# pennneutrinos/chroma

Hardware: AMD Instinct MI355X
Metric: photons/sec (propagate_hit) (higher is better)
Workload: dtype f32

## Files before the change

### chroma_amd/csrc/chroma_hip.hip

```cpp
#include <hip/hip_runtime.h>
#include <stdint.h>
#include <stdio.h>
#include <stdarg.h>
#include <stdlib.h>
#include <string.h>
#include <string>
#include <vector>
#include <algorithm>
#include <chrono>
#include <atomic>
#include <mutex>
#include <unordered_map>
#include <map>

#include <dlfcn.h>
#include <rccl/rccl.h>

#ifndef CHROMA_EXPERIMENTAL
#define CHROMA_EXPERIMENTAL 0
#endif
#include "propagate_device.h"
#include "wide_build.h"
#include "host_utils.h"

// ... 466 lines not shown
{
    const uint32_t i = blockIdx.x * blockDim.x + threadIdx.x;
    if (i >= nnodes) return;
    uint4 n = nodes[i];
    if ((n.w >> CHROMA_CHILD_BITS) == 0) { const uint32_t t = n.w & ~CHROMA_NCHILD_MASK; n.w = t < ntriangles ? tri_to_dev[t] : n.w; }
    out[i] = n;
}
__global__ void k_triangle_records(const float *vertices, const uint32_t *triangles, const uint32_t *codes, const uint32_t *rank,
                                   const uint32_t *dev_to_tri, uint32_t nrecords, float4 *tri)
{
    const uint32_t k = blockIdx.x * blockDim.x + threadIdx.x;
    if (k >= nrecords) return;
    const uint32_t t = dev_to_tri[k];
    const uint32_t extra[3] = {codes[t], t, rank[t]};
#pragma unroll
    for (int c = 0; c < 3; c++) {
        const float *vv = vertices + 3 * (size_t)triangles[3 * (size_t)t + c];
        tri[(size_t)TRI_STRIDE * k + c] = make_float4(vv[0], vv[1], vv[2], __uint_as_float(extra[c]));
    }
}
__global__ void k_triangle_phys(GeoView g, uint32_t nrecords, uint4 *out)
{
    const uint32_t k = blockIdx.x * blockDim.x + threadIdx.x;
    if (k >= nrecords) return;
    const float4 *t = g.tri + (size_t)TRI_STRIDE * k;
    const float4 a = t[0], b = t[1], c = t[2];
    const v3 v0 = mk3(a.x, a.y, a.z), v1 = mk3(b.x, b.y, b.z), v2 = mk3(c.x, c.y, c.z);
    const v3 n = triangle_normal(v0, v1, v2);
    uint32_t bx, by, bz;
    leaf_words(g, v0, v1, v2, bx, by, bz);
    out[2 * (size_t)k] = make_uint4(__float_as_uint(n.x), __float_as_uint(n.y), __float_as_uint(n.z), __float_as_uint(a.w));
    out[2 * (size_t)k + 1] = make_uint4(__float_as_uint(b.w), bx, by, bz);
}
__global__ void k_stack_need_ref(const uint4 *nodes, uint32_t nnodes, uint32_t *need, uint32_t *changed)
{
    const uint32_t i = blockIdx.x * blockDim.x + threadIdx.x;
    if (i >= nnodes) return;
    const uint32_t w = nodes[i].w, nchild = w >> CHROMA_CHILD_BITS, first = w & ~CHROMA_NCHILD_MASK;
    if (nchild == 0) return;
    uint32_t best = 0;
    if ((uint64_t)first + nchild > nnodes || first <= i) best = 0xFFFFu;
    else {
        uint32_t rank = 0;
        for (uint32_t j = 0; j < nchild; j++)
            if ((nodes[first + j].w >> CHROMA_CHILD_BITS) != 0) { best = max(best, rank + need[first + j]); rank++; }
        best = min(max(best, rank), 0xFFFFu);
    }
    if (best != need[i]) { need[i] = best; *changed = 1u; }
}
__global__ void k_stack_need_wide(const uint4 *wnodes, uint32_t nwide, uint32_t *need, uint32_t *changed)
{
    const uint32_t i = blockIdx.x * blockDim.x + threadIdx.x;
    if (i >= nwide) return;
    uint32_t inner = 0, below = 0;
    for (int j = 0; j < 8; j++) {
        const uint32_t w = wnodes[8 * (size_t)i + j].w;
        if (w == 0xFFFFFFFFu || (w & 0x80000000u)) continue;
        inner++;
        if (w < nwide && w > i) below = max(below, need[w]);
    }
    const uint32_t v = min(0xFFFFu, inner ? inner - 1u + below : 0u);
    if (v != need[i]) { need[i] = v; *changed = 1u; }
}
template <class Pass>
static int stack_need_fixed_point(chroma_ctx *ctx, size_t n, Pass pass, uint32_t *result)
{
// ... 629 lines not shown
        void *dtri = nullptr;
        size_t bytes = nrecords * (16 * TRI_STRIDE);
        hipError_t e = ctx_malloc(ctx, &dtri, bytes);
        if (e != hipSuccess) { chroma_geometry_destroy(g); return set_error((int)e, "hipMalloc(%zu) for triangle records: %s", bytes, hipGetErrorString(e)); }
        g->allocations.push_back(dtri);
        g->device_bytes += bytes;
        uint32_t *d_rank = nullptr;
        e = ctx_malloc(ctx, (void **)&d_rank, std::max<size_t>(d->ntriangles, 1) * 4);
        if (e != hipSuccess) { chroma_geometry_destroy(g); return set_error((int)e, "hipMalloc for triangle ranks: %s", hipGetErrorString(e)); }
        rc = chroma_internal_htod(ctx, d_rank, tri_rank, (size_t)d->ntriangles * 4);
        if (rc == CHROMA_OK) {
            hipLaunchKernelGGL(k_triangle_records, dim3((unsigned)((nrecords + 255) / 256)), dim3(256), 0, ctx->stream, (const float *)g->d_vertices, (const uint32_t *)g->d_triangles,
                               (const uint32_t *)g->d_material_codes, d_rank, v.dev_to_tri, (uint32_t)nrecords, (float4 *)dtri);
            e = hipStreamSynchronize(ctx->stream);
            if (e != hipSuccess) rc = set_error((int)e, "triangle records: %s", hipGetErrorString(e));
        }
        hipFree(d_rank);
        if (rc != CHROMA_OK) { chroma_geometry_destroy(g); return rc; }
        v.tri = (const float4 *)dtri;
    }
    {
        void *dphys = nullptr;
        size_t bytes = std::max<size_t>(nrecords, 1) * 32;
        hipError_t e = ctx_malloc(ctx, &dphys, bytes);
        if (e != hipSuccess) { chroma_geometry_destroy(g); return set_error((int)e, "hipMalloc(%zu) for physics records: %s", bytes, hipGetErrorString(e)); }
        g->allocations.push_back(dphys);
        g->device_bytes += bytes;
        if (nrecords) hipLaunchKernelGGL(k_triangle_phys, dim3((unsigned)((nrecords + 255) / 256)), dim3(256), 0, ctx->stream, v, (uint32_t)nrecords, (uint4 *)dphys);
        e = hipStreamSynchronize(ctx->stream);
        if (e == hipSuccess) e = hipGetLastError();
        if (e != hipSuccess) { chroma_geometry_destroy(g); return set_error((int)e, "physics records: %s", hipGetErrorString(e)); }
        v.tri_phys = (const uint4 *)dphys;
    }
    phase("triangle records");
    { const uint32_t *p; if ((rc = upload(g, d->colors, d->colors ? d->ntriangles : 0, &p)) != CHROMA_OK) { chroma_geometry_destroy(g); return rc; } g->d_colors = (void *)p; }
    UP(solid_id_map, d->solid_id_map, d->solid_id_map ? d->ntriangles : 0);
    size_t wn = d->wavelength_n;
    UP(mat_refractive_index, d->mat_refractive_index, d->nmaterials * wn);
    UP(mat_absorption_length, d->mat_absorption_length, d->nmaterials * wn);
    UP(mat_scattering_length, d->mat_scattering_length, d->nmaterials * wn);
    UP(mat_num_comp, d->mat_num_comp, d->nmaterials);
    UP(mat_comp_offset, d->mat_comp_offset, d->nmaterials);
    UP(comp_reemission_prob, d->comp_reemission_prob, d->ncomp_total * wn);
    UP(comp_reemission_wvl_cdf, d->comp_reemission_wvl_cdf, d->ncomp_total * wn);
    UP(comp_absorption_length, d->comp_absorption_length, d->ncomp_total * wn);
    UP(comp_reemission_time_cdf, d->comp_reemission_time_cdf, (size_t)d->ncomp_total * d->time_n);
    UP(surf_detect, d->surf_detect, d->nsurfaces * wn);
    UP(surf_absorb, d->surf_absorb, d->nsurfaces * wn);
    UP(surf_reemit, d->surf_reemit, d->nsurfaces * wn);
    UP(surf_reflect_diffuse, d->surf_reflect_diffuse, d->nsurfaces * wn);
    UP(surf_reflect_specular, d->surf_reflect_specular, d->nsurfaces * wn);
    UP(surf_eta, d->surf_eta, d->nsurfaces * wn);
    UP(surf_k, d->surf_k, d->nsurfaces * wn);
    UP(surf_reemission_cdf, d->surf_reemission_cdf, d->nsurfaces * wn);
    {
        std::vector<SurfaceInfo> info(std::max<uint32_t>(d->nsurfaces, 1));
        for (uint32_t s = 0; s < d->nsurfaces; s++)
            info[s] = SurfaceInfo{d->surf_model[s], d->surf_transmissive[s], d->surf_thickness[s],
                                  d->surf_dichroic_index ? d->surf_dichroic_index[s] : -1};
        UP(surf_info, info.data(), info.size());
    }
    UP(dichroic_nangles, d->dichroic_nangles, d->ndichroic);
    UP(dichroic_offset, d->dichroic_offset, d->ndichroic);
    UP(dichroic_angles, d->dichroic_angles, d->ndichroic_angles_total);
    UP(dichroic_reflect, d->dichroic_reflect, d->ndichroic_angles_total * wn);
    UP(dichroic_transmit, d->dichroic_transmit, d->ndichroic_angles_total * wn);
// ... 33 lines not shown
    if (g->stack_need > STACK_LDS + STACK_SCRATCH) {
        uint32_t need = g->stack_need;
        chroma_geometry_destroy(g);
        return set_error(CHROMA_ERR_STACK, "BVH needs %u traversal stack entries, more than the %d supported", need, STACK_LDS + STACK_SCRATCH);
    }
    *out = g;
    return CHROMA_OK;
}

int chroma_geometry_destroy(chroma_geometry *g)
{
    if (!g) return CHROMA_OK;
    hipSetDevice(g->ctx->device);
    hipStreamSynchronize(g->ctx->stream);
    for (void *p : g->allocations) hipFree(p);
    delete g;
    return CHROMA_OK;
}

int chroma_geometry_device_ptr(chroma_geometry *g, const char *name, void **d_ptr, size_t *nbytes)
{
    if (!g || !name || !d_ptr) return set_error(CHROMA_ERR_INVALID, "bad argument");
    std::string n(name);
    size_t bytes = 0; void *p = nullptr;
    if (n == "nodes") { p = g->d_nodes_api; bytes = g->nnodes * 16; }
    else if (n == "vertices") { p = g->d_vertices; bytes = g->nvertices * 12; }
    else if (n == "triangles") { p = g->d_triangles; bytes = g->ntriangles * 12; }
    else if (n == "material_codes") { p = g->d_material_codes; bytes = g->ntriangles * 4; }
    else if (n == "colors") { p = g->d_colors; bytes = g->ntriangles * 4; }
    else if (n == "solid_id_map") { p = (void *)g->view.solid_id_map; bytes = g->ntriangles * 4; }
    else if (n == "solid_id_to_channel_index") { p = (void *)g->view.solid_id_to_channel_index; bytes = (size_t)g->view.nsolids * 4; }
    else if (n == "triangle_records") { p = (void *)g->view.tri; bytes = g->nrecords * (16 * TRI_STRIDE); }
    else if (n == "triangle_phys") { p = (void *)g->view.tri_phys; bytes = g->nrecords * 32; }
    else if (n == "wide_nodes") { p = (void *)g->view.wnodes; bytes = g->nwide * 128; }
    else if (n == "tri_to_dev") { p = (void *)g->view.tri_to_dev; bytes = g->ntriangles * 4; }
    else if (n == "dev_to_tri") { p = (void *)g->view.dev_to_tri; bytes = g->nrecords * 4; }
    else return set_error(CHROMA_ERR_INVALID, "unknown geometry array '%s'", name);
    *d_ptr = p;
    if (nbytes) *nbytes = bytes;
    return CHROMA_OK;
}

int chroma_geometry_stack_need(chroma_geometry *g, uint32_t *entries)
{
    if (!g || !entries) return set_error(CHROMA_ERR_INVALID, "bad argument");
    *entries = g->stack_need;
    return CHROMA_OK;
}

int chroma_propagate_step(chroma_ctx *ctx, chroma_geometry *geom, int32_t first_photon, int32_t nthreads,
                          const uint32_t *d_input_queue, uint32_t *d_output_queue, chroma_rng rng,
                          const chroma_photon_arrays *photons, int32_t max_steps, int32_t use_weights,
                          int32_t scatter_first)
{
    if (!ctx || !geom) return set_error(CHROMA_ERR_INVALID, "bad argument");
    int rc = check_photons(photons, true);
    if (rc) return rc;
    if (first_photon < 0 || nthreads < 0) return set_error(CHROMA_ERR_INVALID, "negative photon range");
    return launch_propagate(ctx, call_opts(ctx), geom, to_view(photons), first_photon, nthreads, d_input_queue, d_output_queue, rng,
                            max_steps, use_weights, scatter_first);
}

int chroma_photon_duplicate(chroma_ctx *ctx, int32_t first_photon, int32_t nthreads,
                            const chroma_photon_arrays *photons, int32_t copies, int32_t stride)
{
    if (!ctx) return set_error(CHROMA_ERR_INVALID, "null ctx");
// ... 908 lines not shown
```

### chroma_amd/csrc/device_common.h

```cpp
#pragma once

#include <hip/hip_runtime.h>
#include <stdint.h>

#define CM_FN __host__ __device__ static inline
#include "../../include/chroma_math.h"
#include "../../include/chroma_hip.h"

#define WAVE 64

struct v3 { float x, y, z; };
__device__ inline v3 mk3(float x, float y, float z) { return v3{x, y, z}; }
__device__ inline v3 operator-(v3 a) { return mk3(-a.x, -a.y, -a.z); }
__device__ inline v3 operator+(v3 a, v3 b) { return mk3(a.x + b.x, a.y + b.y, a.z + b.z); }
__device__ inline v3 operator-(v3 a, v3 b) { return mk3(a.x - b.x, a.y - b.y, a.z - b.z); }
__device__ inline v3 operator*(v3 a, float c) { return mk3(a.x * c, a.y * c, a.z * c); }
__device__ inline v3 operator*(float c, v3 a) { return mk3(c * a.x, c * a.y, c * a.z); }
__device__ inline v3 operator/(v3 a, float c) { return mk3(a.x / c, a.y / c, a.z / c); }
__device__ inline v3 operator/(v3 a, v3 b) { return mk3(a.x / b.x, a.y / b.y, a.z / b.z); }
__device__ inline v3 operator/(float c, v3 a) { return mk3(c / a.x, c / a.y, c / a.z); }
__device__ inline float dot(v3 a, v3 b) { return a.x * b.x + a.y * b.y + a.z * b.z; }
__device__ inline v3 cross(v3 a, v3 b)
{ return mk3(a.y * b.z - a.z * b.y, a.z * b.x - a.x * b.z, a.x * b.y - a.y * b.x); }
__device__ inline float norm(v3 a) { return cm_sqrtf(dot(a, a)); }
__device__ inline v3 normalize(v3 a) { return a / norm(a); }

__device__ inline v3 load3(const float *p, size_t i) { return mk3(p[3 * i], p[3 * i + 1], p[3 * i + 2]); }
__device__ inline void store3(float *p, size_t i, v3 v) { p[3 * i] = v.x; p[3 * i + 1] = v.y; p[3 * i + 2] = v.z; }

struct SurfaceInfo { uint32_t model; uint32_t transmissive; float thickness; int32_t dichroic_index; };

#ifndef TRI_STRIDE
#define TRI_STRIDE 3
#endif
struct GeoView {
    const uint4  *nodes;
    const uint4  *wnodes;
    const float4 *tri;
    const uint4  *tri_phys;
    const uint32_t *tri_to_dev, *dev_to_tri;
    const float *mat_refractive_index, *mat_absorption_length, *mat_scattering_length;
    const uint32_t *mat_num_comp, *mat_comp_offset;
    const float *comp_reemission_prob, *comp_reemission_wvl_cdf, *comp_absorption_length, *comp_reemission_time_cdf;
    const float *surf_detect, *surf_absorb, *surf_reemit, *surf_reflect_diffuse, *surf_reflect_specular,
                *surf_eta, *surf_k, *surf_reemission_cdf;
    const SurfaceInfo *surf_info;
    const uint32_t *dichroic_nangles, *dichroic_offset;
    const float *dichroic_angles, *dichroic_reflect, *dichroic_transmit;
    const uint32_t *solid_id_map;
    const int32_t  *solid_id_to_channel_index;
    float world_origin[3];
    float world_scale;
    float suspect_margin;
    float slab_grow;
    uint32_t wavelength_n; float wavelength_start, wavelength_step;
    uint32_t time_n;       float time_start, time_step;
    uint32_t nnodes, ntriangles, nsolids, nchannels, nwide;
    uint32_t plain_optics;
};

struct TriPhys { v3 normal; uint32_t code, id, bx, by, bz; };
__device__ inline TriPhys load_tri_phys(const GeoView &g, size_t record)
{
    const uint4 *r = g.tri_phys + 2 * record;
    const uint4 a = r[0], b = r[1];
    return TriPhys{mk3(__uint_as_float(a.x), __uint_as_float(a.y), __uint_as_float(a.z)), a.w, b.x, b.y, b.z, b.w};
}

struct PhotonView {
    float *pos, *dir, *pol, *wavelengths, *t;
    uint32_t *flags; int32_t *last_hit_triangles; float *weights; uint32_t *evidx; uint32_t *rng_counters;
// ... 67 lines not shown
```

### chroma_amd/csrc/kernel_raycast_literal.h

```cpp
#pragma once

#ifndef LIT_STACK
#define LIT_STACK 32
#endif
#define LIT_STRIDE (LIT_STACK + 1)
#ifndef LIT_TRI_MIN
#define LIT_TRI_MIN 8
#endif
#ifndef LIT_TRI_END_HALF
#define LIT_TRI_END_HALF 1
#endif
#ifndef LIT_REFILL_MIN
#define LIT_REFILL_MIN 4
#endif
#ifndef LIT_WAVES_PER_EU
#define LIT_WAVES_PER_EU 8
#endif
#ifndef LIT_DIAG
#define LIT_DIAG 0
#endif
#define LIT_SPILL (2 * COOP_SPILL)

template <int K>
__device__ inline uint32_t quad_bcast_u32(uint32_t v)
// ... 135 lines not shown
                const float tmin = box_tmin_exact(nd, ws, wox, woy, woz, inv_dir, noid);
                const bool pass = valid && node_passes(tmin, min_distance);
                const bool leaf = (nd.w >> CHROMA_CHILD_BITS) == 0u;
                const bool is_tri = pass && leaf && (int)(nd.w & ~CHROMA_NCHILD_MASK) != last_hit;
                const bool is_inner = pass && !leaf;
                const uint32_t qm = quad_or_u32((is_inner ? (jbit << 4) : 0u) | (is_tri ? jbit : 0u));
                if ((qm & 0xFu) == 0u) {
                    const uint32_t mi = qm >> 4;
                    const int pos = sp + (int)__popc(mi & below);
                    if (is_inner) {
                        if (pos < LIT_STACK) stack[pos] = nd.w;
                        else if (pos < LIT_STACK + LIT_SPILL) { spill[pos - LIT_STACK] = nd.w; if (COUNT) cnt.spills++; }
                    }
                    sp += (int)__popc(mi);
                    if (sp > LIT_STACK + LIT_SPILL) { if (j == 0) cnt.overflows++; sp = LIT_STACK + LIT_SPILL; }
                } else {
                    waiting = true;
                    w_node = nd.w;
                    w_tmin = tmin;
                    w_qm = qm;
                }
            }
        } while ((int)__popcll(__ballot(waiting) & 0x1111111111111111ull) < tri_min &&
                 (int)__popcll(__ballot(active && !waiting) & 0x1111111111111111ull) > stop_at);
        __builtin_amdgcn_s_setprio(0);

        if (__any(waiting)) {
#if LIT_DIAG
            if (COUNT) { diag_passes++; diag_waiting += (unsigned)__popcll(__ballot(waiting) & 0x1111111111111111ull); }
#endif
            bool hit = false;
            float distance = 0.0f;
            if (waiting && (w_qm & jbit)) {
                const float4 *tp = g.tri + TRI_STRIDE * (size_t)(w_node & ~CHROMA_NCHILD_MASK);
                const float4 a = tp[0], b = tp[1], c = tp[2];
                hit = intersect_triangle(origin, direction, mk3(a.x, a.y, a.z), mk3(b.x, b.y, b.z), mk3(c.x, c.y, c.z), distance);
            }
            const uint32_t hm = quad_or_u32(hit ? jbit : 0u);
            if (waiting) {
                const float t0 = quad_bcast_f32<0>(w_tmin), t1 = quad_bcast_f32<1>(w_tmin), t2 = quad_bcast_f32<2>(w_tmin), t3 = quad_bcast_f32<3>(w_tmin);
                const float d0 = quad_bcast_f32<0>(distance), d1 = quad_bcast_f32<1>(distance), d2 = quad_bcast_f32<2>(distance), d3 = quad_bcast_f32<3>(distance);
                float m = min_distance;
                uint32_t win = 4u, acc = 0u, ntested = 0u;
#define LIT_REPLAY(K, TK, DK)                                                                                          \
                if ((w_qm & (0x11u << K)) && node_passes(TK, m)) {                                                     \
                    if (w_qm & (1u << K)) {                                                                            \
                        ntested++;                                                                                     \
                        if ((hm & (1u << K)) && (m < 0.0f || DK < m)) { m = DK; win = K; }               \
                    } else {                                                                                           \
                        acc |= 1u << K;                                                                                \
                    }                                                                                                  \
                }
                LIT_REPLAY(0, t0, d0) LIT_REPLAY(1, t1, d1) LIT_REPLAY(2, t2, d2) LIT_REPLAY(3, t3, d3)
#undef LIT_REPLAY
                if (COUNT && j == 0) cnt.tris += ntested;
                const uint32_t wchild = quad_max_u32(j == win ? (w_node & ~CHROMA_NCHILD_MASK) + 1u : 0u);
                if (win != 4u) { triangle_index = (int)wchild - 1; min_distance = m; }
                if (acc) {
                    const int pos = sp + (int)__popc(acc & below);
                    if (acc & jbit) {
                        if (pos < LIT_STACK) stack[pos] = w_node;
                        else if (pos < LIT_STACK + LIT_SPILL) { spill[pos - LIT_STACK] = w_node; if (COUNT) cnt.spills++; }
                    }
                    sp += (int)__popc(acc);
                    if (sp > LIT_STACK + LIT_SPILL) { if (j == 0) cnt.overflows++; sp = LIT_STACK + LIT_SPILL; }
                }
            }
            waiting = false;
            __builtin_amdgcn_wave_barrier();
// ... 45 lines not shown
                              cm_fabsf(noid.x) < 1e30f && cm_fabsf(noid.y) < 1e30f && cm_fabsf(noid.z) < 1e30f;
        if (!moderate) triangle_index = HIT_RETRY; else active = true;
    }
    uint32_t cur = 0, end = 1;
    int sp = 0;
    while (__any(active)) {
        if (active && cur >= end) {
            if (sp == 0) {
                active = false;
            } else {
                sp--;
                const uint32_t w = (sp < LIT_STACK) ? stack[sp] : spill[sp - LIT_STACK];
                cur = w & ~CHROMA_NCHILD_MASK;
                end = cur + (w >> CHROMA_CHILD_BITS);
            }
        }
        if (active) {
            const uint32_t idx = cur + j;
            const bool valid = idx < end;
            const uint4 nd = g.nodes[valid ? idx : end - 1u];
            if (COUNT && j8 == 0 && end != 1u) cnt.nodes += min(4u, end - cur);
            cur += 4u;
            const float tmin = box_tmin_exact(nd, ws, wox, woy, woz, inv_dir, noid);
            const bool pass = valid && node_passes(tmin, min_distance);
            const bool leaf = (nd.w >> CHROMA_CHILD_BITS) == 0u;
            const bool is_tri = pass && leaf && (int)(nd.w & ~CHROMA_NCHILD_MASK) != last_hit;
            const bool is_inner = pass && !leaf;
            const uint32_t qm = quad_or_u32((is_inner ? (jbit << 4) : 0u) | (is_tri ? jbit : 0u));
            uint32_t acc = qm >> 4;
            if (qm & 0xFu) {
                bool hit = false;
                float distance = 0.0f;
                if (is_tri) {
                    const float4 *tp = g.tri + TRI_STRIDE * (size_t)(nd.w & ~CHROMA_NCHILD_MASK);
                    const float4 a = tp[0], b = tp[1], c = tp[2];
                    hit = intersect_triangle(origin, direction, mk3(a.x, a.y, a.z), mk3(b.x, b.y, b.z), mk3(c.x, c.y, c.z), distance);
                }
                const uint32_t hm = quad_or_u32(hit ? jbit : 0u);
                const float t0 = quad_bcast_f32<0>(tmin), t1 = quad_bcast_f32<1>(tmin), t2 = quad_bcast_f32<2>(tmin), t3 = quad_bcast_f32<3>(tmin);
                const float d0 = quad_bcast_f32<0>(distance), d1 = quad_bcast_f32<1>(distance), d2 = quad_bcast_f32<2>(distance), d3 = quad_bcast_f32<3>(distance);
                float m = min_distance;
                uint32_t win = 4u, ntested = 0u;
                acc = 0u;
#define LIT_REPLAY(K, TK, DK)                                                                                          \
                if ((qm & (0x11u << K)) && node_passes(TK, m)) {                                                       \
                    if (qm & (1u << K)) {                                                                              \
                        ntested++;                                                                                     \
                        if ((hm & (1u << K)) && (m < 0.0f || DK < m)) { m = DK; win = K; }               \
                    } else {                                                                                           \
                        acc |= 1u << K;                                                                                \
                    }                                                                                                  \
                }
                LIT_REPLAY(0, t0, d0) LIT_REPLAY(1, t1, d1) LIT_REPLAY(2, t2, d2) LIT_REPLAY(3, t3, d3)
#undef LIT_REPLAY
                if (COUNT && j8 == 0) cnt.tris += ntested;
                const uint32_t wchild = quad_max_u32(j == win ? (nd.w & ~CHROMA_NCHILD_MASK) + 1u : 0u);
                if (win != 4u) { triangle_index = (int)wchild - 1; min_distance = m; }
            }
            if (acc) {
                const int pos = sp + (int)__popc(acc & below);
                if ((acc & jbit) && j8 < 4u) {
                    if (pos < LIT_STACK) stack[pos] = nd.w;
                    else if (pos < LIT_STACK + LIT_SPILL) { spill[pos - LIT_STACK] = nd.w; if (COUNT) cnt.spills++; }
                }
                sp += (int)__popc(acc);
                if (sp > LIT_STACK + LIT_SPILL) { if (j8 == 0) cnt.overflows++; sp = LIT_STACK + LIT_SPILL; }
            }
            __builtin_amdgcn_wave_barrier();
        }
// ... 4 lines not shown
```

### chroma_amd/csrc/kernel_raycast_quad.h

```cpp
#pragma once

#ifndef QUAD_PENDING
#define QUAD_PENDING 16
#endif
#ifndef QUAD_STACK
#define QUAD_STACK COOP_STACK
#endif
#define QUAD_OD_WORDS 6
#define QUAD_STRIDE (2 * QUAD_STACK + QUAD_PENDING + QUAD_OD_WORDS + 1)
#ifndef QUAD_REFILL_MIN
#define QUAD_REFILL_MIN 4
#endif
#ifndef QUAD_WAVES_PER_EU
#define QUAD_WAVES_PER_EU 8
#endif
#ifndef QUAD_TIMING
#define QUAD_TIMING 0
#endif
#ifndef QUAD_FLUSH
#define QUAD_FLUSH 8
#endif
#ifndef QUAD_KEEP
#define QUAD_KEEP 7
#endif

__device__ inline uint32_t quad_min_u32(uint32_t v)
{
    v = min(v, (uint32_t)__builtin_amdgcn_update_dpp(0, (int)v, 0xB1, 0xF, 0xF, false));
    v = min(v, (uint32_t)__builtin_amdgcn_update_dpp(0, (int)v, 0x4E, 0xF, 0xF, false));
    return v;
}
__device__ inline uint32_t quad_max_u32(uint32_t v)
{
    v = max(v, (uint32_t)__builtin_amdgcn_update_dpp(0, (int)v, 0xB1, 0xF, 0xF, false));
    v = max(v, (uint32_t)__builtin_amdgcn_update_dpp(0, (int)v, 0x4E, 0xF, 0xF, false));
    return v;
}

typedef float f32x2 __attribute__((ext_vector_type(2)));
__device__ inline void box_interval_pk(float ax, float ay, float az, f32x2 bx, f32x2 by, f32x2 bz, uint4 nd, float &tmin, float &tmax)
{
    f32x2 qx = {(float)(nd.x & 0xFFFFu), (float)(nd.x >> 16)};
    f32x2 qy = {(float)(nd.y & 0xFFFFu), (float)(nd.y >> 16)};
    f32x2 qz = {(float)(nd.z & 0xFFFFu), (float)(nd.z >> 16)};
    const f32x2 tx = __builtin_elementwise_fma(qx, (f32x2){ax, ax}, bx);
    const f32x2 ty = __builtin_elementwise_fma(qy, (f32x2){ay, ay}, by);
    const f32x2 tz = __builtin_elementwise_fma(qz, (f32x2){az, az}, bz);
    tmin = __builtin_fmaxf(__builtin_fmaxf(__builtin_fminf(tx.x, tx.y), __builtin_fminf(ty.x, ty.y)),
                           __builtin_fmaxf(__builtin_fminf(tz.x, tz.y), 0.0f));
    tmax = __builtin_fminf(__builtin_fminf(__builtin_fmaxf(tx.x, tx.y), __builtin_fmaxf(ty.x, ty.y)),
                           __builtin_fmaxf(tz.x, tz.y));
}
__device__ inline void box_interval_signed(float ax, float ay, float az, uint32_t sx, uint32_t sy, uint32_t sz,
                                           f32x2 bx, f32x2 by, f32x2 bz, uint4 nd, float &tmin, float &tmax)
{
    const uint32_t x = __builtin_amdgcn_alignbit(nd.x, nd.x, sx), y = __builtin_amdgcn_alignbit(nd.y, nd.y, sy),
                   z = __builtin_amdgcn_alignbit(nd.z, nd.z, sz);
    f32x2 qx = {(float)(x & 0xFFFFu), (float)(x >> 16)};
    f32x2 qy = {(float)(y & 0xFFFFu), (float)(y >> 16)};
    f32x2 qz = {(float)(z & 0xFFFFu), (float)(z >> 16)};
    const f32x2 tx = __builtin_elementwise_fma(qx, (f32x2){ax, ax}, bx);
    const f32x2 ty = __builtin_elementwise_fma(qy, (f32x2){ay, ay}, by);
    const f32x2 tz = __builtin_elementwise_fma(qz, (f32x2){az, az}, bz);
    tmin = __builtin_fmaxf(__builtin_fmaxf(tx.x, ty.x), __builtin_fmaxf(tz.x, 0.0f));
    tmax = __builtin_fminf(__builtin_fminf(tx.y, ty.y), tz.y);
}
__device__ inline uint32_t quad_or_u32(uint32_t v)
{
    v |= (uint32_t)__builtin_amdgcn_update_dpp(0, (int)v, 0xB1, 0xF, 0xF, false);
    v |= (uint32_t)__builtin_amdgcn_update_dpp(0, (int)v, 0x4E, 0xF, 0xF, false);
    return v;
}
// ... 35 lines not shown
    uint32_t cur = WIDE_NONE;
    int sp = 0, npend = 0;
    uint32_t phead = 0;
    uint32_t loc_next = 0, loc_end = 0;
    bool exhausted = false;
#if QUAD_TIMING
    unsigned long long tq_refill = 0, tq_pop = 0, tq_wait = 0, tq_node = 0, tq_leaf = 0, tq_retire = 0, tq_a, tq_b;
    unsigned tq_iters = 0, tq_rounds = 0, tq_outer = 0, tq_active = 0, tq_tests = 0;
#define TQ_STAMP(v) asm volatile("s_memtime %0\n\ts_waitcnt lgkmcnt(0)" : "=s"(v) :: "memory")
    const unsigned long long tq_start = __builtin_readcyclecounter();
#endif

    for (;;) {
#if QUAD_TIMING
        TQ_STAMP(tq_a); tq_outer++;
#endif
        unsigned long long idle_mask = __ballot(!has_ray && j == 0);
        int n_idle = __popcll(idle_mask);
        bool more = !exhausted || loc_next < loc_end;
        if (more && (n_idle >= QUAD_REFILL_MIN || n_idle == 16)) {
            if (loc_next >= loc_end) {
                const uint32_t base = wc.next(work_counter, lane, exhausted);
                loc_next = min(base, (uint32_t)nthreads);
                loc_end = min(base + (uint32_t)chunk, (uint32_t)nthreads);
            }
            uint32_t idx = loc_next + (uint32_t)__popcll(idle_mask & ((1ull << gshift) - 1ull));
            loc_next = min(loc_end, loc_next + (uint32_t)n_idle);
            if (!has_ray && idx < loc_end) {
                slot = first_photon + (int)idx;
                const float4 *r = rays + 4 * (size_t)slot;
                const float4 r0 = r[0], r1 = r[1];
                if (__float_as_int(r1.w) == 0) {
                    const float4 r2 = r[2], r3 = r[3];
                    if (j == 0) { ray_od[0] = r0.x; ray_od[1] = r0.y; ray_od[2] = r0.z; ray_od[3] = r1.x; ray_od[4] = r1.y; ray_od[5] = r1.z; }
                    { const int lh = __float_as_int(r0.w); last_hit_w = lh >= 0 ? (0x80000000u | (uint32_t)lh) : WIDE_NONE; }
                    rax = r2.x; ray_ = r2.y; raz = r2.z;
                    { const float mx = r2.w * cm_fabsf(rax), my = r2.w * cm_fabsf(ray_), mz = r2.w * cm_fabsf(raz);
                      rbx = (f32x2){r3.x - mx, r3.x + mx}; rby = (f32x2){r3.y - my, r3.y + my}; rbz = (f32x2){r3.z - mz, r3.z + mz}; }
                    rsx = rax < 0.f ? 16u : 0u; rsy = ray_ < 0.f ? 16u : 0u; rsz = raz < 0.f ? 16u : 0u;
                    triangle_index = -1;
                    prune_t = cm_inff();
                    sp = 0;
                    npend = 0;
                    phead = 0;
                    cur = 0;
                    has_ray = true;
                    active = true;
                } else if (settle && j == 0) {
                    const int status = __float_as_int(r1.w);
                    hit_triangle[slot] = status;
                    hit_distance[slot] = 0.0f;
                    if (status == HIT_RETRY) retry_list[atomicAdd(retry_counter, 1u)] = (uint32_t)slot;
                }
            }
        }
        if (!__any(has_ray)) {
            if (exhausted && loc_next >= loc_end) break;
            continue;
        }

#if QUAD_TIMING
        TQ_STAMP(tq_b); tq_refill += tq_b - tq_a;
#endif
        more = !exhausted || loc_next < loc_end;
        const int stop_at = more ? max(0, (int)__popcll(__ballot(active) & 0x1111111111111111ull) - (int)QUAD_REFILL_MIN) : 0;
        do {
#if QUAD_TIMING
// ... 62 lines not shown
                            if (pos < QUAD_STACK) { stack_n[pos] = ea.w; stack_t[pos] = ta; }
                            else if (pos < QUAD_STACK + COOP_SPILL) { spill[pos - QUAD_STACK] = make_uint2(ea.w, __float_as_uint(ta)); if (COUNT) atomicAdd(&counters->stack_spills, 1ull); }
                            pos++;
                        }
                        if (qb) {
                            if (pos < QUAD_STACK) { stack_n[pos] = eb.w; stack_t[pos] = tb; }
                            else if (pos < QUAD_STACK + COOP_SPILL) { spill[pos - QUAD_STACK] = make_uint2(eb.w, __float_as_uint(tb)); if (COUNT) atomicAdd(&counters->stack_spills, 1ull); }
                        }
                        if (sp > QUAD_STACK + COOP_SPILL) { atomicAdd(&counters->stack_overflows, 1ull); sp = QUAD_STACK + COOP_SPILL; }
                    }
                }
            }
#if QUAD_TIMING
            TQ_STAMP(tq_b); tq_node += tq_b - tq_a;
#endif
        } while (!__any(npend >= QUAD_FLUSH) && (int)__popcll(__ballot(active) & 0x1111111111111111ull) > stop_at);
        __builtin_amdgcn_wave_barrier();
#if QUAD_TIMING
        TQ_STAMP(tq_a);
#endif

        while (__any(npend > (active ? QUAD_KEEP : 0))) {
#if QUAD_TIMING
            tq_rounds++; tq_tests += (unsigned)__popcll(__ballot(npend > 0 && (int)j < min(npend, 4)));
#endif
            {
                const int take = min(npend, 4);
                bool hit = false;
                float distance = 0.0f;
                uint32_t tri = 0, rank = 0xFFFFFFFFu;
                if ((int)j < take) tri = pending[(phead + j) & (QUAD_PENDING - 1u)];
                if ((int)j < take && (0x80000000u | tri) != last_hit_w) {
                    if (COUNT) cnt.tris++;
                    const float4 *tp = g.tri + TRI_STRIDE * (size_t)tri;
                    float4 a = tp[0], b = tp[1], c = tp[2];
                    const v3 origin = mk3(ray_od[0], ray_od[1], ray_od[2]), direction = mk3(ray_od[3], ray_od[4], ray_od[5]);
                    hit = intersect_triangle(origin, direction, mk3(a.x, a.y, a.z), mk3(b.x, b.y, b.z), mk3(c.x, c.y, c.z), distance);
                    rank = __float_as_uint(c.w);
                }
                const uint32_t dkey = hit ? __float_as_uint(distance) : 0x7F800000u;
                const uint32_t dmin = quad_min_u32(dkey);
                const float dm = __uint_as_float(dmin);
                const bool cand = hit && dkey == dmin;
                const uint32_t rm = quad_min_u32(cand ? rank : 0xFFFFFFFFu);
                const uint32_t wtri = quad_max_u32((cand && rank == rm) ? tri + 1u : 0u) - 1u;
                const bool better = dmin != 0x7F800000u && (dm < prune_t || (dm == prune_t && rm < best_rank));
                triangle_index = better ? (int)wtri : triangle_index;
                prune_t = better ? dm : prune_t;
                best_rank = better ? rm : best_rank;
                phead = (phead + (uint32_t)take) & (QUAD_PENDING - 1u);
                npend -= take;
            }
        }


#if QUAD_TIMING
        TQ_STAMP(tq_b); tq_leaf += tq_b - tq_a;
#endif
        if (has_ray && !active) {
            if (j == 0) {
                hit_triangle[slot] = triangle_index;
                hit_distance[slot] = triangle_index == -1 ? -1.0f : prune_t;
                if (triangle_index == HIT_RETRY) retry_list[atomicAdd(retry_counter, 1u)] = (uint32_t)slot;
            }
            has_ray = false;
        }
    }

#if QUAD_TIMING
    if (lane == 0 && (blockIdx.x & 1023u) == 0u && nthreads > 1000000) {
        const unsigned long long total = __builtin_readcyclecounter() - tq_start;
// ... 13 lines not shown
```

### chroma_amd/csrc/kernel_tail_coop.h

```cpp
#pragma once

template <bool COUNT>
__device__ inline int coop_cast(const GeoView &g, v3 origin, v3 direction, int last_hit, bool on, float &min_distance,
                                uint32_t *stack_n, float *stack_t, uint32_t *pending, uint2 *spill,
                                unsigned j, unsigned gshift, uint32_t below, LaneCounters &cnt)
{
    const float inf = cm_inff();
    int triangle_index = -1;
    uint32_t best_rank = 0;
    min_distance = -1.0f;
    uint32_t cur = WIDE_NONE;
    int sp = 0, npend = 0;
    bool active = false;
    RayFast rf;
    rf.a = rf.blo = rf.bhi = mk3(0.f, 0.f, 0.f);
    if (on) {
        v3 noid = (-origin) / direction;
        v3 inv_dir = 1.0f / direction;
        bool moderate = cm_fabsf(inv_dir.x) < 1e30f && cm_fabsf(inv_dir.y) < 1e30f && cm_fabsf(inv_dir.z) < 1e30f &&
                        cm_fabsf(noid.x) < 1e30f && cm_fabsf(noid.y) < 1e30f && cm_fabsf(noid.z) < 1e30f;
        if (!moderate) {
            triangle_index = HIT_RETRY;
        } else {
            rf = ray_fast(g, noid, inv_dir, ray_growth(g, origin));
// ... 26 lines not shown
                const uint32_t gi = (uint32_t)(__ballot(inner) >> gshift) & 0xFFu;
                if (leaf) pending[npend + __popc(gl & below)] = w & 0x7FFFFFFFu;
                npend += __popc(gl);
                cur = WIDE_NONE;
                if (gi) {
                    const float tm = group8_min(inner ? t : inf);
                    const uint32_t gn = (uint32_t)(__ballot(inner && t == tm) >> gshift) & 0xFFu;
                    const uint32_t nj = (uint32_t)__ffs((int)gn) - 1u;
                    const uint32_t others = gi & ~(1u << nj);
                    if (inner && j != nj) {
                        int pos = sp + __popc(others & below);
                        if (pos < COOP_STACK) { stack_n[pos] = w; stack_t[pos] = t; }
                        else if (pos < COOP_STACK + COOP_SPILL) { spill[pos - COOP_STACK] = make_uint2(w, __float_as_uint(t)); if (COUNT) cnt.spills++; }
                    }
                    sp += __popc(others);
                    cur = (uint32_t)__shfl((int)w, (int)(gshift + nj));
                    if (sp > COOP_STACK + COOP_SPILL) {
                        triangle_index = HIT_RETRY;
                        active = false; npend = 0; cur = WIDE_NONE; sp = 0;
                    }
                }
            }
        }
        __builtin_amdgcn_wave_barrier();
        while (__any(npend > 0)) {
            if (npend > 0) {
                const int take = min(npend, 8);
                bool hit = false;
                float distance = inf;
                uint32_t tri = 0, rank = 0xFFFFFFFFu;
                if ((int)j < take) {
                    tri = pending[j];
                    if (COUNT) cnt.tris++;
                    const float4 *tp = g.tri + TRI_STRIDE * (size_t)tri;
                    float4 a = tp[0], b = tp[1], c = tp[2];
                    hit = intersect_triangle(origin, direction, mk3(a.x, a.y, a.z), mk3(b.x, b.y, b.z), mk3(c.x, c.y, c.z), distance);
                    rank = __float_as_uint(c.w);
                }
                const float dm = group8_min(hit ? distance : inf);
                if (dm < inf) {
                    const bool cand = hit && distance == dm;
                    const uint32_t rm = group8_min_u32(cand ? rank : 0xFFFFFFFFu);
                    const uint32_t gw = (uint32_t)(__ballot(cand && rank == rm) >> gshift) & 0xFFu;
                    const uint32_t wj = (uint32_t)__ffs((int)gw) - 1u;
                    const int wtri = __shfl((int)tri, (int)(gshift + wj));
                    if (triangle_index == -1 || dm < min_distance || (dm == min_distance && rm < best_rank)) {
                        triangle_index = wtri;
                        min_distance = dm;
                        best_rank = rm;
                    }
                }
                if (npend > 8) {
                    uint32_t mv = pending[j + 8];
                    if ((int)j + 8 < npend) pending[j] = mv;
                }
                npend -= take;
            }
        }
        __builtin_amdgcn_wave_barrier();
    }
    return triangle_index;
}

template <bool COUNT, bool LITERAL = false>
__global__ __launch_bounds__(PROP_BLOCK) void
k_tail_coop(GeoView g, PhotonView pv, const StepState *st, const float4 *work_in,
            uint64_t seed, uint64_t id_base, int max_steps, int use_weights, int scatter_first, uint2 *spill_base,
            DeviceCounters *counters, HitsOut h, uint32_t *words)
{
    __shared__ uint32_t s_coop[8 * COOP_STRIDE];
// ... 138 lines not shown
```

### chroma_amd/csrc/propagate_device.h

```cpp
#pragma once
#include "device_common.h"
#include <float.h>

#define WEIGHT_LOWER_THRESHOLD 0.0001f
#define CHROMA_EPSILON 1e-6
enum { CMD_BREAK = 0, CMD_CONTINUE = 1, CMD_PASS = 2 };

struct Photon {
    v3 position, direction, polarization;
    float wavelength, time, weight;
    uint32_t history;
    int last_hit_triangle;
    uint32_t evidx;
};

struct State {
    v3 surface_normal;
    float refractive_index1, refractive_index2;
    float absorption_length, scattering_length;
    int material1;
    int surface_index;
    float distance_to_boundary;
};

// ... 4 lines not shown
    float start = g.wavelength_start, step = g.wavelength_step;
    uint32_t n = g.wavelength_n;
    if (x < start) return fp[0];
    if (x > (start + (float)(n - 1) * step)) return fp[n - 1];
    int jl = cm_f2i((x - start) / step);
    int ju = (jl + 1 < (int)n) ? jl + 1 : (int)n - 1;
    return fp[jl] + (x - (start + (float)jl * step)) * (fp[ju] - fp[jl]) / step;
}
__device__ inline const float *row(const float *tab, const GeoView &g, int idx) { return tab + (size_t)idx * g.wavelength_n; }

#define MT_NEG_EPS  __uint_as_float(0xB58637BDu)
#define MT_ONE_EPS  __uint_as_float(0x3F800008u)
#define MT_POS_EPS  __uint_as_float(0x358637BDu)
__device__ inline bool intersect_triangle(v3 origin, v3 direction, v3 v0, v3 v1, v3 v2, float &distance)
{
    v3 edge1 = v1 - v0;
    v3 edge2 = v2 - v0;
    v3 h = cross(direction, edge2);
    float a = dot(edge1, h);
    if (a > -FLT_EPSILON && a < FLT_EPSILON) return false;
    float f = 1.0f / a;
    v3 s = origin - v0;
    float u = f * dot(s, h);
    if (u < MT_NEG_EPS || u > MT_ONE_EPS) return false;
    v3 q = cross(s, edge1);
    float v = f * dot(direction, q);
    if (v < MT_NEG_EPS || (u + v) > MT_ONE_EPS) return false;
    float t = f * dot(edge2, q);
    if (t > MT_POS_EPS && t < cm_inff()) {
        distance = t;
        return true;
    }
    return false;
}

__device__ inline float box_tmin(v3 origin, v3 noid, v3 inv_dir, v3 lower, v3 upper, float ws)
{
    float tmin = 0.0f, tmax = cm_inff();
    float t0, t1;
    if (cm_isfinite(inv_dir.x)) {
        t0 = lower.x * inv_dir.x + noid.x;
        t1 = upper.x * inv_dir.x + noid.x;
        tmin = cm_fmaxf(tmin, cm_fminf(t0, t1));
        tmax = cm_fminf(tmax, cm_fmaxf(t0, t1));
    } else if (origin.x < lower.x - ws || origin.x > upper.x + ws) return -1.0f;
    if (cm_isfinite(inv_dir.y)) {
        t0 = lower.y * inv_dir.y + noid.y;
        t1 = upper.y * inv_dir.y + noid.y;
        tmin = cm_fmaxf(tmin, cm_fminf(t0, t1));
        tmax = cm_fminf(tmax, cm_fmaxf(t0, t1));
    } else if (origin.y < lower.y - ws || origin.y > upper.y + ws) return -1.0f;
    if (cm_isfinite(inv_dir.z)) {
        t0 = lower.z * inv_dir.z + noid.z;
        t1 = upper.z * inv_dir.z + noid.z;
        tmin = cm_fmaxf(tmin, cm_fminf(t0, t1));
        tmax = cm_fminf(tmax, cm_fmaxf(t0, t1));
    } else if (origin.z < lower.z - ws || origin.z > upper.z + ws) return -1.0f;
    if (tmin > tmax) return -1.0f;
    return tmin;
}

__device__ inline bool reference_tests_leaf(const GeoView &g, uint32_t bx, uint32_t by, uint32_t bz, v3 origin, v3 direction, float t)
{
    const float ws = g.world_scale;
    const v3 noid = (-origin) / direction;
    const v3 inv_dir = 1.0f / direction;
// ... 140 lines not shown
    int triangle_index = -1;
    min_distance = -1.0f;
    if (!lane_on) return -1;
    const v3 noid = (-origin) / direction;
    const v3 inv_dir = 1.0f / direction;
    const v3 wo = mk3(g.world_origin[0], g.world_origin[1], g.world_origin[2]);
    const float ws = g.world_scale;
#define S_LO(nd) mk3(wo.x + (float)((nd).x & 0xFFFFu) * ws, wo.y + (float)((nd).y & 0xFFFFu) * ws, wo.z + (float)((nd).z & 0xFFFFu) * ws)
#define S_HI(nd) mk3(wo.x + (float)((nd).x >> 16) * ws, wo.y + (float)((nd).y >> 16) * ws, wo.z + (float)((nd).z >> 16) * ws)
    TravStack<LDS_N, BLOCK> stack;
    stack.lds = lds;
    uint4 root = g.nodes[0];
    if (!node_passes(box_tmin(origin, noid, inv_dir, S_LO(root), S_HI(root), ws), min_distance)) return -1;
    int sp = 0;
    stack.put(sp++, root.w);
    while (sp > 0) {
        uint32_t w = stack.get(--sp);
        uint32_t first = w & ~CHROMA_NCHILD_MASK, n = w >> CHROMA_CHILD_BITS;
        for (uint32_t i0 = first; i0 < first + n; i0 += 4) {
            const uint32_t last = first + n - 1;
            uint4 quad[4];
#pragma unroll
            for (int k = 0; k < 4; k++) quad[k] = g.nodes[min(i0 + (uint32_t)k, last)];
#pragma unroll
            for (int k = 0; k < 4; k++) {
                if (i0 + (uint32_t)k > last) break;
                const uint4 nd = quad[k];
                if (COUNT) cnt.nodes++;
                if (!node_passes(box_tmin(origin, noid, inv_dir, S_LO(nd), S_HI(nd), ws), min_distance)) continue;
                uint32_t child = nd.w & ~CHROMA_NCHILD_MASK;
                if ((nd.w >> CHROMA_CHILD_BITS) == 0) {
                    if ((int)child == last_hit_record) continue;
                    if (COUNT) cnt.tris++;
                    const float4 *t = g.tri + TRI_STRIDE * (size_t)child;
                    float4 a = t[0], b = t[1], c = t[2];
                    float distance;
                    if (intersect_triangle(origin, direction, mk3(a.x, a.y, a.z), mk3(b.x, b.y, b.z), mk3(c.x, c.y, c.z), distance)) {
                        if (triangle_index == -1 || distance < min_distance) {
                            triangle_index = (int)child;
                            min_distance = distance;
                        }
                    }
                } else if (sp >= LDS_N + STACK_SCRATCH) {
                    cnt.overflows++;
                    return triangle_index;
                } else {
                    stack.put(sp++, nd.w);
                }
            }
        }
    }
#undef S_LO
#undef S_HI
    return triangle_index;
}

template <int LDS_N, int BLOCK, bool COUNT>
__device__ inline int intersect_mesh(const GeoView &g, v3 origin, v3 direction, float &min_distance,
                                     int last_hit_triangle, uint32_t *lds, LaneCounters &cnt, bool lane_on = true)
{
    int last_hit_dev = (lane_on && last_hit_triangle >= 0) ? (int)g.tri_to_dev[last_hit_triangle] : -1;
    int found = intersect_mesh_strict<LDS_N, BLOCK, COUNT>(g, origin, direction, min_distance, last_hit_dev, lds, cnt, lane_on);
    return (found >= 0) ? (int)g.dev_to_tri[found] : found;
}
template <int LDS_N, int BLOCK, bool COUNT>
__device__ inline int intersect_mesh_dev(const GeoView &g, v3 origin, v3 direction, float &min_distance,
                                         int last_hit_dev, uint32_t *lds, LaneCounters &cnt, bool lane_on = true)
{
    return intersect_mesh_strict<LDS_N, BLOCK, COUNT>(g, origin, direction, min_distance, last_hit_dev, lds, cnt, lane_on);
}
// ... 611 lines not shown
```

Before: 853.8 million.

## Precompute triangle edge records and use packed-f32 Möller-Trumbore intersection

Adds a build-time kernel that stores each triangle as precomputed edges e1/e2 interleaved per axis plus v0 and rank in a 48-byte record. All ray-triangle tests in the traversal kernels now read these records and run a branchless intersection on two-wide float vectors, pairing origin and direction components so the hardware can use packed FMA. The goal is fewer subtractions and less instruction issue per triangle test. The cost is an extra device buffer per geometry and a slightly different order of floating-point operations.

```diff
diff --git a/chroma_amd/csrc/chroma_hip.hip b/chroma_amd/csrc/chroma_hip.hip
--- a/chroma_amd/csrc/chroma_hip.hip
+++ b/chroma_amd/csrc/chroma_hip.hip
@@ -522,6 +522,17 @@
     out[2 * (size_t)k] = make_uint4(__float_as_uint(n.x), __float_as_uint(n.y), __float_as_uint(n.z), __float_as_uint(a.w));
     out[2 * (size_t)k + 1] = make_uint4(__float_as_uint(b.w), bx, by, bz);
 }
+__global__ void k_triangle_isect(GeoView g, uint32_t nrecords, float4 *out)
+{
+    const uint32_t k = blockIdx.x * blockDim.x + threadIdx.x;
+    if (k >= nrecords) return;
+    const float4 *t = g.tri + (size_t)TRI_STRIDE * k;
+    const float4 a = t[0], b = t[1], c = t[2];
+    const v3 v0 = mk3(a.x, a.y, a.z), e1 = mk3(b.x, b.y, b.z) - v0, e2 = mk3(c.x, c.y, c.z) - v0;
+    out[3 * (size_t)k] = make_float4(e1.x, e2.x, e1.y, e2.y);
+    out[3 * (size_t)k + 1] = make_float4(e1.z, e2.z, v0.x, v0.y);
+    out[3 * (size_t)k + 2] = make_float4(v0.z, c.w, 0.0f, 0.0f);
+}
 __global__ void k_stack_need_ref(const uint4 *nodes, uint32_t nnodes, uint32_t *need, uint32_t *changed)
 {
     const uint32_t i = blockIdx.x * blockDim.x + threadIdx.x;
@@ -1217,6 +1228,19 @@
         if (e != hipSuccess) { chroma_geometry_destroy(g); return set_error((int)e, "physics records: %s", hipGetErrorString(e)); }
         v.tri_phys = (const uint4 *)dphys;
     }
+    {
+        void *disect = nullptr;
+        size_t bytes = std::max<size_t>(nrecords, 1) * 48;
+        hipError_t e = ctx_malloc(ctx, &disect, bytes);
+        if (e != hipSuccess) { chroma_geometry_destroy(g); return set_error((int)e, "hipMalloc(%zu) for intersection records: %s", bytes, hipGetErrorString(e)); }
+        g->allocations.push_back(disect);
+        g->device_bytes += bytes;
+        if (nrecords) hipLaunchKernelGGL(k_triangle_isect, dim3((unsigned)((nrecords + 255) / 256)), dim3(256), 0, ctx->stream, v, (uint32_t)nrecords, (float4 *)disect);
+        e = hipStreamSynchronize(ctx->stream);
+        if (e == hipSuccess) e = hipGetLastError();
+        if (e != hipSuccess) { chroma_geometry_destroy(g); return set_error((int)e, "intersection records: %s", hipGetErrorString(e)); }
+        v.tri_isect = (const float4 *)disect;
+    }
     phase("triangle records");
     { const uint32_t *p; if ((rc = upload(g, d->colors, d->colors ? d->ntriangles : 0, &p)) != CHROMA_OK) { chroma_geometry_destroy(g); return rc; } g->d_colors = (void *)p; }
     UP(solid_id_map, d->solid_id_map, d->solid_id_map ? d->ntriangles : 0);
@@ -1316,6 +1340,7 @@
     else if (n == "solid_id_to_channel_index") { p = (void *)g->view.solid_id_to_channel_index; bytes = (size_t)g->view.nsolids * 4; }
     else if (n == "triangle_records") { p = (void *)g->view.tri; bytes = g->nrecords * (16 * TRI_STRIDE); }
     else if (n == "triangle_phys") { p = (void *)g->view.tri_phys; bytes = g->nrecords * 32; }
+    else if (n == "triangle_isect") { p = (void *)g->view.tri_isect; bytes = g->nrecords * 48; }
     else if (n == "wide_nodes") { p = (void *)g->view.wnodes; bytes = g->nwide * 128; }
     else if (n == "tri_to_dev") { p = (void *)g->view.tri_to_dev; bytes = g->ntriangles * 4; }
     else if (n == "dev_to_tri") { p = (void *)g->view.dev_to_tri; bytes = g->nrecords * 4; }
diff --git a/chroma_amd/csrc/device_common.h b/chroma_amd/csrc/device_common.h
--- a/chroma_amd/csrc/device_common.h
+++ b/chroma_amd/csrc/device_common.h
@@ -8,6 +8,8 @@
 #include "../../include/chroma_hip.h"
 
 #define WAVE 64
+
+typedef float f32x2 __attribute__((ext_vector_type(2)));
 
 struct v3 { float x, y, z; };
 __device__ inline v3 mk3(float x, float y, float z) { return v3{x, y, z}; }
@@ -37,6 +39,7 @@
     const uint4  *nodes;
     const uint4  *wnodes;
     const float4 *tri;
+    const float4 *tri_isect;
     const uint4  *tri_phys;
     const uint32_t *tri_to_dev, *dev_to_tri;
     const float *mat_refractive_index, *mat_absorption_length, *mat_scattering_length;
diff --git a/chroma_amd/csrc/kernel_raycast_literal.h b/chroma_amd/csrc/kernel_raycast_literal.h
--- a/chroma_amd/csrc/kernel_raycast_literal.h
+++ b/chroma_amd/csrc/kernel_raycast_literal.h
@@ -191,9 +191,7 @@
             bool hit = false;
             float distance = 0.0f;
             if (waiting && (w_qm & jbit)) {
-                const float4 *tp = g.tri + TRI_STRIDE * (size_t)(w_node & ~CHROMA_NCHILD_MASK);
-                const float4 a = tp[0], b = tp[1], c = tp[2];
-                hit = intersect_triangle(origin, direction, mk3(a.x, a.y, a.z), mk3(b.x, b.y, b.z), mk3(c.x, c.y, c.z), distance);
+                hit = intersect_triangle_edges(origin, direction, g.tri_isect + 3 * (size_t)(w_node & ~CHROMA_NCHILD_MASK), distance);
             }
             const uint32_t hm = quad_or_u32(hit ? jbit : 0u);
             if (waiting) {
@@ -305,9 +303,7 @@
                 bool hit = false;
                 float distance = 0.0f;
                 if (is_tri) {
-                    const float4 *tp = g.tri + TRI_STRIDE * (size_t)(nd.w & ~CHROMA_NCHILD_MASK);
-                    const float4 a = tp[0], b = tp[1], c = tp[2];
-                    hit = intersect_triangle(origin, direction, mk3(a.x, a.y, a.z), mk3(b.x, b.y, b.z), mk3(c.x, c.y, c.z), distance);
+                    hit = intersect_triangle_edges(origin, direction, g.tri_isect + 3 * (size_t)(nd.w & ~CHROMA_NCHILD_MASK), distance);
                 }
                 const uint32_t hm = quad_or_u32(hit ? jbit : 0u);
                 const float t0 = quad_bcast_f32<0>(tmin), t1 = quad_bcast_f32<1>(tmin), t2 = quad_bcast_f32<2>(tmin), t3 = quad_bcast_f32<3>(tmin);
diff --git a/chroma_amd/csrc/kernel_raycast_quad.h b/chroma_amd/csrc/kernel_raycast_quad.h
--- a/chroma_amd/csrc/kernel_raycast_quad.h
+++ b/chroma_amd/csrc/kernel_raycast_quad.h
@@ -37,7 +37,6 @@
     return v;
 }
 
-typedef float f32x2 __attribute__((ext_vector_type(2)));
 __device__ inline void box_interval_pk(float ax, float ay, float az, f32x2 bx, f32x2 by, f32x2 bz, uint4 nd, float &tmin, float &tmax)
 {
     f32x2 qx = {(float)(nd.x & 0xFFFFu), (float)(nd.x >> 16)};
@@ -139,7 +138,7 @@
                 const float4 r0 = r[0], r1 = r[1];
                 if (__float_as_int(r1.w) == 0) {
                     const float4 r2 = r[2], r3 = r[3];
-                    if (j == 0) { ray_od[0] = r0.x; ray_od[1] = r0.y; ray_od[2] = r0.z; ray_od[3] = r1.x; ray_od[4] = r1.y; ray_od[5] = r1.z; }
+                    if (j == 0) { ray_od[0] = r0.x; ray_od[1] = r1.x; ray_od[2] = r0.y; ray_od[3] = r1.y; ray_od[4] = r0.z; ray_od[5] = r1.z; }
                     { const int lh = __float_as_int(r0.w); last_hit_w = lh >= 0 ? (0x80000000u | (uint32_t)lh) : WIDE_NONE; }
                     rax = r2.x; ray_ = r2.y; raz = r2.z;
                     { const float mx = r2.w * cm_fabsf(rax), my = r2.w * cm_fabsf(ray_), mz = r2.w * cm_fabsf(raz);
@@ -268,11 +267,8 @@
                 if ((int)j < take) tri = pending[(phead + j) & (QUAD_PENDING - 1u)];
                 if ((int)j < take && (0x80000000u | tri) != last_hit_w) {
                     if (COUNT) cnt.tris++;
-                    const float4 *tp = g.tri + TRI_STRIDE * (size_t)tri;
-                    float4 a = tp[0], b = tp[1], c = tp[2];
-                    const v3 origin = mk3(ray_od[0], ray_od[1], ray_od[2]), direction = mk3(ray_od[3], ray_od[4], ray_od[5]);
-                    hit = intersect_triangle(origin, direction, mk3(a.x, a.y, a.z), mk3(b.x, b.y, b.z), mk3(c.x, c.y, c.z), distance);
-                    rank = __float_as_uint(c.w);
+                    hit = intersect_triangle_edges((f32x2){ray_od[0], ray_od[1]}, (f32x2){ray_od[2], ray_od[3]}, (f32x2){ray_od[4], ray_od[5]},
+                                                   g.tri_isect + 3 * (size_t)tri, distance, rank);
                 }
                 const uint32_t dkey = hit ? __float_as_uint(distance) : 0x7F800000u;
                 const uint32_t dmin = quad_min_u32(dkey);
diff --git a/chroma_amd/csrc/kernel_tail_coop.h b/chroma_amd/csrc/kernel_tail_coop.h
--- a/chroma_amd/csrc/kernel_tail_coop.h
+++ b/chroma_amd/csrc/kernel_tail_coop.h
@@ -82,10 +82,8 @@
                 if ((int)j < take) {
                     tri = pending[j];
                     if (COUNT) cnt.tris++;
-                    const float4 *tp = g.tri + TRI_STRIDE * (size_t)tri;
-                    float4 a = tp[0], b = tp[1], c = tp[2];
-                    hit = intersect_triangle(origin, direction, mk3(a.x, a.y, a.z), mk3(b.x, b.y, b.z), mk3(c.x, c.y, c.z), distance);
-                    rank = __float_as_uint(c.w);
+                    hit = intersect_triangle_edges((f32x2){origin.x, direction.x}, (f32x2){origin.y, direction.y}, (f32x2){origin.z, direction.z},
+                                                   g.tri_isect + 3 * (size_t)tri, distance, rank);
                 }
                 const float dm = group8_min(hit ? distance : inf);
                 if (dm < inf) {
diff --git a/chroma_amd/csrc/propagate_device.h b/chroma_amd/csrc/propagate_device.h
--- a/chroma_amd/csrc/propagate_device.h
+++ b/chroma_amd/csrc/propagate_device.h
@@ -60,6 +60,34 @@
         return true;
     }
     return false;
+}
+
+__device__ inline bool intersect_triangle_edges(f32x2 rx, f32x2 ry, f32x2 rz, const float4 *rec, float &distance, uint32_t &rank)
+{
+    const float4 w0 = rec[0], w1 = rec[1], w2 = rec[2];
+    const f32x2 ex = {w0.x, w0.y}, ey = {w0.z, w0.w}, ez = {w1.x, w1.y};
+    const f32x2 sx = {rx.x - w1.z, rx.y}, sy = {ry.x - w1.w, ry.y}, sz = {rz.x - w2.x, rz.y};
+    rank = __float_as_uint(w2.y);
+    const f32x2 qx = sy * ez - sz * ey, qy = sz * ex - sx * ez, qz = sx * ey - sy * ex;
+    const f32x2 at = (ex * qx.yx + ey * qy.yx) + ez * qz.yx;
+    const f32x2 uv = (sx * qx.yx + sy * qy.yx) + sz * qz.yx;
+    const float a = at.x;
+    const float f = 1.0f / a;
+    const f32x2 w = (f32x2){f, f} * uv;
+    const float u = w.x, v = w.y, t = f * at.y;
+    const bool hit = !(a > -FLT_EPSILON && a < FLT_EPSILON) & !(u < MT_NEG_EPS || u > MT_ONE_EPS) &
+                     !(v < MT_NEG_EPS || (u + v) > MT_ONE_EPS) & (t > MT_POS_EPS && t < cm_inff());
+    distance = t;
+    return hit;
+}
+__device__ inline bool intersect_triangle_edges(v3 origin, v3 direction, const float4 *rec, float &distance)
+{
+    uint32_t rank;
+    float t;
+    const bool hit = intersect_triangle_edges((f32x2){origin.x, direction.x}, (f32x2){origin.y, direction.y},
+                                              (f32x2){origin.z, direction.z}, rec, t, rank);
+    if (hit) distance = t;
+    return hit;
 }
 
 __device__ inline float box_tmin(v3 origin, v3 noid, v3 inv_dir, v3 lower, v3 upper, float ws)
@@ -266,10 +294,8 @@
                 if ((nd.w >> CHROMA_CHILD_BITS) == 0) {
                     if ((int)child == last_hit_record) continue;
                     if (COUNT) cnt.tris++;
-                    const float4 *t = g.tri + TRI_STRIDE * (size_t)child;
-                    float4 a = t[0], b = t[1], c = t[2];
                     float distance;
-                    if (intersect_triangle(origin, direction, mk3(a.x, a.y, a.z), mk3(b.x, b.y, b.z), mk3(c.x, c.y, c.z), distance)) {
+                    if (intersect_triangle_edges(origin, direction, g.tri_isect + 3 * (size_t)child, distance)) {
                         if (triangle_index == -1 || distance < min_distance) {
                             triangle_index = (int)child;
                             min_distance = distance;
```

New measurement: 890.6 million, median of 6. 4.3% higher.
